# applied-ai-lab/genesis

Hardware: AMD Instinct MI355X
Metric: training images/sec (fwd+bwd+GECO step), GENESIS-V2 K=7 64x64 (higher is better)
Workload: dtype f32

## Files before the change

### genesis_amd/csrc/gx_wino.hip

```cpp
#include <stdlib.h>

#include "gx_common.h"

namespace {

constexpr int WKC = 8;
constexpr int WTH = 4, WTW = 8;
constexpr int WNT = WTH * WTW;
constexpr int PR = 2 * WTH + 2, PC = 2 * WTW + 2;
constexpr int PLANE = 10;
constexpr int PPITCH = PR * 2 * PLANE;
constexpr int RAW_FLOATS = WKC * PPITCH;
constexpr int V_FLOATS = 16 * WKC * WNT;
constexpr int RAW_PER_THREAD = (WKC * PR * PC + 255) / 256;

struct WinoGeom {
    int N, K, M;
    int K1, M1;
    int Kpad, Mpad;
    int H, W;
    int tiles_h, tiles_w;
    const float* xam0; const float* xam1;
    int xn0, xn1;
};
// ... 224 lines not shown
#pragma unroll
        for (int a = 0; a < 4; ++a)
#pragma unroll
            for (int b = 0; b < 2; ++b)
#pragma unroll
                for (int c = 0; c < 16; ++c) sacc += acc[a][b][c];
        outp[out_n + (size_t)(m0 - mbase + (tid >> 2)) * HW + (size_t)R0 * g.W + C0 + (tid & 3)] = sacc;
        return;
    }
#pragma unroll
    for (int mi = 0; mi < 2; ++mi) {
        __syncthreads();
#pragma unroll
        for (int r4 = 0; r4 < 4; ++r4)
#pragma unroll
            for (int e = 0; e < 4; ++e) {
                const int row = e + 8 * r4 + 4 * kh;
                const int rg = 4 * r4 + e;
                const float q0 = acc[0][mi][rg] + acc[1][mi][rg] + acc[2][mi][rg];
                const float q1 = acc[1][mi][rg] - acc[2][mi][rg] - acc[3][mi][rg];
                E[((wave * 2 + 0) * 32 + row) * 32 + bn] = q0;
                E[((wave * 2 + 1) * 32 + row) * 32 + bn] = q1;
            }
        __syncthreads();
#pragma unroll
        for (int j = 0; j < 4; ++j) {
            const int ml = (tid >> 5) + 8 * j;
            const int m = m0 + mi * 32 + ml;
            if (m >= g.M) continue;
            const int ty = tt >> 3, tx = tt & 7;
            float q[4][2];
#pragma unroll
            for (int xi = 0; xi < 4; ++xi) {
                q[xi][0] = E[((xi * 2 + 0) * 32 + ml) * 32 + tt];
                q[xi][1] = E[((xi * 2 + 1) * 32 + ml) * 32 + tt];
            }
            float2 y0, y1;
            y0.x = q[0][0] + q[1][0] + q[2][0];
            y0.y = q[0][1] + q[1][1] + q[2][1];
            y1.x = q[1][0] - q[2][0] - q[3][0];
            y1.y = q[1][1] - q[2][1] - q[3][1];
            float* o = outp + out_n + (size_t)(m - mbase) * HW + (size_t)(R0 + 2 * ty) * g.W + C0 + 2 * tx;
            *reinterpret_cast<float2*>(o) = y0;
            *reinterpret_cast<float2*>(o + g.W) = y1;
        }
    }
}

#ifndef GX_WH_ABL
#define GX_WH_ABL 0
#endif
constexpr int HKC = 16;
typedef __bf16 w_bf16x8 __attribute__((ext_vector_type(8)));
typedef float w_f32x16 __attribute__((ext_vector_type(16)));

__device__ __forceinline__ void wino_split8(const float (&v)[8], w_bf16x8& ph, w_bf16x8& pm, w_bf16x8& pl) {
#pragma unroll
    for (int e = 0; e < 8; ++e) {
        const __bf16 h = (__bf16)v[e];
        const float r1 = v[e] - (float)h;
        const __bf16 m = (__bf16)r1;
        ph[e] = h; pm[e] = m; pl[e] = (__bf16)(r1 - (float)m);
    }
}

typedef _Float16 w_f16x8 __attribute__((ext_vector_type(8)));
typedef float w_f32x2 __attribute__((ext_vector_type(2)));
typedef _Float16 w_f16x2 __attribute__((ext_vector_type(2)));
typedef unsigned w_u32x4 __attribute__((ext_vector_type(4)));
__device__ __forceinline__ void wino_split8_f16(const float (&v)[8], float sc, w_bf16x8& ph, w_bf16x8& pl) {
    w_u32x4 h, l;
#pragma unroll
    for (int i = 0; i < 4; ++i) {
        const float s0 = v[2 * i] * sc, s1 = v[2 * i + 1] * sc;
        const float h0 = __builtin_bit_cast(float, __builtin_bit_cast(unsigned, s0) & 0xFFFFE000u);
        const float h1 = __builtin_bit_cast(float, __builtin_bit_cast(unsigned, s1) & 0xFFFFE000u);
        h[i] = __builtin_bit_cast(unsigned, __builtin_convertvector(w_f32x2{h0, h1}, w_f16x2));
        l[i] = __builtin_bit_cast(unsigned, __builtin_convertvector(w_f32x2{s0 - h0, s1 - h1}, w_f16x2));
    }
    ph = __builtin_bit_cast(w_bf16x8, h); pl = __builtin_bit_cast(w_bf16x8, l);
}

enum { WPF_B6 = 0, WPF_F3 = 1, WPF_B1 = 2 };
template <int NB, int PF = WPF_B6> struct WHCfg {
    static constexpr int TROWS = 4 * NB;
    static constexpr int PRH = 2 * TROWS + 2;
    static constexpr int USED = PRH * 20;
    static constexpr int PITCH = NB == 1 ? 256 : 384;
    static constexpr int ROUNDS = (USED + 255) / 256;
    static constexpr int RAW_FLOATS = HKC * PITCH;
    static constexpr int NSETS = NB == 1 ? 2 : 4;
    static constexpr int LOOK = NB == 1 ? 1 : 2;
    static constexpr size_t LDS_BYTES = 2 * RAW_FLOATS * 4 > 32768 ? 2 * RAW_FLOATS * 4 : 32768;
    static constexpr int NP = PF == WPF_B1 ? 1 : (PF == WPF_F3 ? 2 : 3);
    static constexpr int POSB = (PF == WPF_B1 ? 1 : 3) * 2048;
};

template <int NB, int PF>
__global__ void __launch_bounds__(256, NB == 1 ? 2 : 1)
wino_conv_h_kernel(const float* __restrict__ in, const float* __restrict__ in2, const unsigned* __restrict__ U,
                   float* __restrict__ out, float* __restrict__ out2, const WinoGeom g) {
    using C = WHCfg<NB, PF>;
    constexpr bool F16 = PF == WPF_F3, B1 = PF == WPF_B1;
    constexpr int NP = C::NP, POSB = C::POSB;
    constexpr int PITCH = C::PITCH, NSETS = C::NSETS, LOOK = C::LOOK;
    extern __shared__ __attribute__((aligned(16))) float lds[];
    float* raw = lds;
    const int tid = threadIdx.x, lane = tid & 63, wave = tid >> 6;

    const int xcd_l = gx_xcd_tile(blockIdx.x + blockIdx.y * gridDim.x, gridDim.x * gridDim.y);
    const int my = xcd_l % (int)gridDim.y;
    int tile = xcd_l / (int)gridDim.y;
    const int tw_i = tile % g.tiles_w; tile /= g.tiles_w;
    const int th_i = tile % g.tiles_h; tile /= g.tiles_h;
    const int n = tile;
    const int R0 = th_i * (2 * C::TROWS), C0 = tw_i * (2 * WTW);
    const int m0 = my * 64;
    const int HW = g.H * g.W;
    const int Ka = g.K1 < g.K ? g.K1 : g.K, Kb = g.K - Ka;
    const float* in_n = in + (size_t)n * Ka * HW;
    const float* in2_n = in2 + (size_t)n * Kb * HW;
    const int nchunks = g.Kpad / HKC;

    int voff[C::ROUNDS];
#pragma unroll
    for (int r = 0; r < C::ROUNDS; ++r) {
        const int p = tid + 256 * r;
        voff[r] = 0x40000000;
        if (p < C::USED) {
            const int pr = p / 20, rem = p - pr * 20, par = rem / 10, idx = rem - par * 10;
            const int rr = R0 - 1 + pr, cc = C0 - 1 + 2 * idx + par;
            if (idx < 9 && rr >= 0 && rr < g.H && cc >= 0 && cc < g.W) voff[r] = (rr * g.W + cc) * 4;
        }
    }
    auto stage = [&](int k0, float* rbuf) {
        const bool second = k0 >= g.K1;
        const int kr = second ? k0 - g.K1 : k0, left = (second ? Kb : Ka) - kr;
        const __amdgpu_buffer_rsrc_t rs = __builtin_amdgcn_make_buffer_rsrc(
            const_cast<float*>((second ? in2_n : in_n) + (size_t)kr * HW), 0, left > 0 ? left * HW * 4 : 0, 0x00020000);
        float* dst = rbuf + __builtin_amdgcn_readfirstlane(wave) * 64;
#pragma unroll
        for (int q = 0; q < HKC; ++q)
#pragma unroll
            for (int r = 0; r < C::ROUNDS; ++r)
                if (r == 0 || wave < (PITCH - 256) / 64)
                    __builtin_amdgcn_raw_ptr_buffer_load_lds(rs, (__attribute__((address_space(3))) void*)(dst + q * PITCH + r * 256),
                                                             4, voff[r] + q * HW * 4, 0, 0, 0);
    };

    const int bn = lane & 31, kh = lane >> 5;
    const int tx = bn & 7;
    const int ra = wave == 0 ? 0 : (wave == 2 ? 2 : 1), rb = wave == 3 ? 3 : (wave == 2 ? 1 : 2);
    const float sgn = wave == 1 ? 1.f : -1.f;
    int ta_off[NB], tb_off[NB];
#pragma unroll
    for (int nb = 0; nb < NB; ++nb) {
        const int ty = (bn >> 3) + 4 * nb;
        ta_off[nb] = (8 * kh) * PITCH + (2 * ty + ra) * 20 + tx;
        tb_off[nb] = (8 * kh) * PITCH + (2 * ty + rb) * 20 + tx;
    }

    const char* Uw = reinterpret_cast<const char*>(U) + ((size_t)my * nchunks * 16 + 4 * wave) * POSB + lane * 16;
    auto load_a = [&](w_bf16x8 (&a)[2][3], int c, int nu) {
        const char* p = Uw + ((size_t)c * 16 + nu) * POSB;
#pragma unroll
        for (int pc = 0; pc < NP; ++pc)
#pragma unroll
            for (int mi = 0; mi < 2; ++mi)
                a[mi][pc] = *reinterpret_cast<const w_bf16x8*>(p + (pc * 2 + mi) * 1024);
    };

    w_f32x16 acc[4][2][NB];
#pragma unroll
    for (int a = 0; a < 4; ++a)
#pragma unroll
        for (int b = 0; b < 2; ++b)
#pragma unroll
            for (int nb = 0; nb < NB; ++nb)
#pragma unroll
                for (int c = 0; c < 16; ++c) acc[a][b][nb][c] = 0.f;

    w_bf16x8 as[NSETS][2][3];
    float scV = 1.f;
    int f16_back = 0;
    if constexpr (F16) {
        float xm = 0.f;
        for (int i = lane; i < g.xn0; i += 64) xm = fmaxf(xm, fabsf(g.xam0[i]));
        for (int i = lane; i < g.xn1; i += 64) xm = fmaxf(xm, fabsf(g.xam1[i]));
#pragma unroll
        for (int of = 32; of >= 1; of >>= 1) xm = fmaxf(xm, __shfl_xor(xm, of, 64));
        const int eV = gx_f16_scale_exp(4.f * xm);
        const float wam = *reinterpret_cast<const float*>(reinterpret_cast<const char*>(U) + gx_kq_h_amax_off(g.Kpad, g.Mpad, 16));
        const int eU = gx_f16_scale_exp(2.25f * wam);
        scV = ldexpf(1.f, eV);
        f16_back = -(eU + eV);
    }
#ifdef GX_WH_STAGGER
    if (((blockIdx.x + gridDim.x * blockIdx.y) >> 8) & 1)
        for (int i = 0; i < GX_WH_STAGGER; ++i) __builtin_amdgcn_s_sleep(1);
#endif
    stage(0, raw);
#pragma unroll
    for (int i = 0; i < LOOK; ++i) load_a(as[i], 0, i);

    for (int c = 0; c < nchunks; ++c) {
        __builtin_amdgcn_s_waitcnt(0x0f70);
        __syncthreads();
        if (c + 1 < nchunks && !(GX_WH_ABL & 8)) stage((c + 1) * HKC, raw + ((c + 1) & 1) * C::RAW_FLOATS);
        const float* rbuf = raw + (c & 1) * C::RAW_FLOATS;
        float t[NB][8][4];
#pragma unroll
        for (int nb = 0; nb < NB; ++nb)
#pragma unroll
            for (int ch = 0; ch < 8; ++ch) {
                const float* pa = rbuf + ta_off[nb] + ch * PITCH;
                const float* pb = rbuf + tb_off[nb] + ch * PITCH;
#pragma unroll
                for (int j = 0; j < 4; ++j) t[nb][ch][j] = fmaf(sgn, pb[(j & 1) * 10 + (j >> 1)], pa[(j & 1) * 10 + (j >> 1)]);
            }
#pragma unroll
        for (int nu = 0; nu < 4; ++nu) {
            w_bf16x8 (&acur)[2][3] = as[nu % NSETS];
            if (!(GX_WH_ABL & 2)) {
                constexpr int dummy = 0; (void)dummy;
                const int pn = nu + LOOK;
                if (pn < 4) load_a(as[pn % NSETS], c, pn);
                else if (c + 1 < nchunks) load_a(as[pn % NSETS], c + 1, pn - 4);
            }
            w_bf16x8 b[NB][3];
#pragma unroll
            for (int nb = 0; nb < NB; ++nb) {
                float v[8];
#pragma unroll
                for (int ch = 0; ch < 8; ++ch)
                    v[ch] = nu == 0 ? t[nb][ch][0] - t[nb][ch][2]
                                    : (nu == 1 ? t[nb][ch][1] + t[nb][ch][2] : (nu == 2 ? t[nb][ch][2] - t[nb][ch][1] : t[nb][ch][1] - t[nb][ch][3]));
                if (GX_WH_ABL & 4) { b[nb][0] = acur[0][0]; b[nb][1] = acur[0][1]; b[nb][2] = acur[0][2]; }
                else if constexpr (B1) {
#pragma unroll
                    for (int e = 0; e < 8; ++e) b[nb][0][e] = (__bf16)v[e];
                }
                else if constexpr (F16) wino_split8_f16(v, scV, b[nb][0], b[nb][1]);
                else wino_split8(v, b[nb][0], b[nb][1], b[nb][2]);
            }
#pragma unroll
            for (int mi = 0; mi < 2; ++mi)
#pragma unroll
                for (int nb = 0; nb < NB; ++nb) {
                    w_f32x16 cc = acc[nu][mi][nb];
                    if (GX_WH_ABL & 1) { cc[0] += (float)acur[mi][0][0] * (float)b[nb][0][0] + (float)acur[mi][1][1] * (float)b[nb][1][1] + (float)acur[mi][2][2] * (float)b[nb][2][2]; acc[nu][mi][nb] = cc; continue; }
                    if constexpr (B1) {
                        acc[nu][mi][nb] = __builtin_amdgcn_mfma_f32_32x32x16_bf16(acur[mi][0], b[nb][0], cc, 0, 0, 0);
                        continue;
                    }
                    if constexpr (F16) {
                        cc = __builtin_amdgcn_mfma_f32_32x32x16_f16(__builtin_bit_cast(w_f16x8, acur[mi][1]), __builtin_bit_cast(w_f16x8, b[nb][0]), cc, 0, 0, 0);
                        cc = __builtin_amdgcn_mfma_f32_32x32x16_f16(__builtin_bit_cast(w_f16x8, acur[mi][0]), __builtin_bit_cast(w_f16x8, b[nb][1]), cc, 0, 0, 0);
                        cc = __builtin_amdgcn_mfma_f32_32x32x16_f16(__builtin_bit_cast(w_f16x8, acur[mi][0]), __builtin_bit_cast(w_f16x8, b[nb][0]), cc, 0, 0, 0);
                        acc[nu][mi][nb] = cc;
                        continue;
                    }
                    cc = __builtin_amdgcn_mfma_f32_32x32x16_bf16(acur[mi][1], b[nb][1], cc, 0, 0, 0);
                    cc = __builtin_amdgcn_mfma_f32_32x32x16_bf16(acur[mi][2], b[nb][0], cc, 0, 0, 0);
                    cc = __builtin_amdgcn_mfma_f32_32x32x16_bf16(acur[mi][0], b[nb][2], cc, 0, 0, 0);
                    cc = __builtin_amdgcn_mfma_f32_32x32x16_bf16(acur[mi][1], b[nb][0], cc, 0, 0, 0);
                    cc = __builtin_amdgcn_mfma_f32_32x32x16_bf16(acur[mi][0], b[nb][1], cc, 0, 0, 0);
                    cc = __builtin_amdgcn_mfma_f32_32x32x16_bf16(acur[mi][0], b[nb][0], cc, 0, 0, 0);
                    acc[nu][mi][nb] = cc;
                }
        }
    }

    float* E = lds;
    const int tt = tid & 31;
    const bool second_out = m0 >= g.M1;
    const int Mo = second_out ? g.M - g.M1 : (g.M1 < g.M ? g.M1 : g.M), mbase = second_out ? g.M1 : 0;
    float* const outp = second_out ? out2 : out;
    const size_t out_n = (size_t)n * Mo * HW;
#pragma unroll
    for (int mi = 0; mi < 2; ++mi)
#pragma unroll
        for (int nb = 0; nb < NB; ++nb) {
            __syncthreads();
#pragma unroll
            for (int r4 = 0; r4 < 4; ++r4)
#pragma unroll
                for (int e = 0; e < 4; ++e) {
                    const int row = e + 8 * r4 + 4 * kh;
                    const int rg = 4 * r4 + e;
                    const float q0 = acc[0][mi][nb][rg] + acc[1][mi][nb][rg] + acc[2][mi][nb][rg];
                    const float q1 = acc[1][mi][nb][rg] - acc[2][mi][nb][rg] - acc[3][mi][nb][rg];
                    E[((wave * 2 + 0) * 32 + row) * 32 + bn] = q0;
                    E[((wave * 2 + 1) * 32 + row) * 32 + bn] = q1;
                }
            __syncthreads();
#pragma unroll
            for (int j = 0; j < 4; ++j) {
                const int ml = (tid >> 5) + 8 * j;
                const int m = m0 + mi * 32 + ml;
                if (m >= g.M) continue;
                const int oy = (tt >> 3) + 4 * nb, ox = tt & 7;
                float q[4][2];
#pragma unroll
                for (int xi = 0; xi < 4; ++xi) {
                    q[xi][0] = E[((xi * 2 + 0) * 32 + ml) * 32 + tt];
                    q[xi][1] = E[((xi * 2 + 1) * 32 + ml) * 32 + tt];
                }
                float2 y0, y1;
                y0.x = q[0][0] + q[1][0] + q[2][0];
                y0.y = q[0][1] + q[1][1] + q[2][1];
                y1.x = q[1][0] - q[2][0] - q[3][0];
                y1.y = q[1][1] - q[2][1] - q[3][1];
                if constexpr (F16) {
                    y0.x = ldexpf(y0.x, f16_back); y0.y = ldexpf(y0.y, f16_back);
                    y1.x = ldexpf(y1.x, f16_back); y1.y = ldexpf(y1.y, f16_back);
                }
                float* o = outp + out_n + (size_t)(m - mbase) * HW + (size_t)(R0 + 2 * oy) * g.W + C0 + 2 * ox;
                *reinterpret_cast<float2*>(o) = y0;
                *reinterpret_cast<float2*>(o + g.W) = y1;
            }
        }
}

__device__ __forceinline__ void wino_h_store(unsigned* __restrict__ U, float v0, float v1, int m, int k, int p, int Kpad16,
                                             bool f16 = false, int f16_exp = 0, bool b1 = false) {
    unsigned short pc[2][3];
    const float v[2] = {v0, v1};
    if (b1) {
        U[gx_wino_h_word(m, k, p, 0, Kpad16, 1)] = (unsigned)__builtin_bit_cast(unsigned short, (__bf16)v0) |
                                                   ((unsigned)__builtin_bit_cast(unsigned short, (__bf16)v1) << 16);
        return;
    }
    if (f16) {
#pragma unroll
        for (int e = 0; e < 2; ++e) {
            const float ws = ldexpf(v[e], f16_exp);
            const _Float16 h = (_Float16)ws;
            pc[e][0] = __builtin_bit_cast(unsigned short, h);
            pc[e][1] = __builtin_bit_cast(unsigned short, (_Float16)(ws - (float)h));
        }
#pragma unroll
        for (int q = 0; q < 2; ++q) U[gx_wino_h_word(m, k, p, q, Kpad16)] = (unsigned)pc[0][q] | ((unsigned)pc[1][q] << 16);
        return;
    }
#pragma unroll
    for (int e = 0; e < 2; ++e) {
        const __bf16 h = (__bf16)v[e];
        const float r1 = v[e] - (float)h;
        const __bf16 mm = (__bf16)r1;
        const __bf16 l = (__bf16)(r1 - (float)mm);
        pc[e][0] = __builtin_bit_cast(unsigned short, h);
        pc[e][1] = __builtin_bit_cast(unsigned short, mm);
        pc[e][2] = __builtin_bit_cast(unsigned short, l);
    }
#pragma unroll
    for (int q = 0; q < 3; ++q) U[gx_wino_h_word(m, k, p, q, Kpad16)] = (unsigned)pc[0][q] | ((unsigned)pc[1][q] << 16);
}

__global__ void wino_pack_h_kernel(const float* __restrict__ w, unsigned* __restrict__ U, int mode, int Co, int Ci, int Kpad16,
                                   int Mpad, const float* __restrict__ amax, int b1) {
    const int total = 16 * (Kpad16 / 2) * Mpad;
    const int f16_exp = amax ? gx_f16_scale_exp(2.25f * *amax) : 0;
    for (int idx = blockIdx.x * blockDim.x + threadIdx.x; idx < total; idx += gridDim.x * blockDim.x) {
        const int m = idx % Mpad, k = 2 * ((idx / Mpad) % (Kpad16 / 2)), p = idx / (Mpad * (Kpad16 / 2));
        wino_h_store(U, gx_wino_u_value(w, mode, Co, Ci, m, k, p), gx_wino_u_value(w, mode, Co, Ci, m, k + 1, p), m, k, p, Kpad16,
                     amax != nullptr, f16_exp, b1 != 0);
    }
}

__global__ void __launch_bounds__(1024)
wino_pair_amax_kernel(const float* __restrict__ w1, const float* __restrict__ w2, int n1, int n2, float* __restrict__ tf,
                      float* __restrict__ td) {
    const float r = gx_wg1024_amax(blockIdx.x == 0 ? w1 : w2, blockIdx.x == 0 ? n1 : n2);
    if (threadIdx.x == 0) { tf[1 + blockIdx.x] = r; td[1 + blockIdx.x] = r; }
}
__global__ void wino_pack_pair_h_kernel(const float* __restrict__ w1, const float* __restrict__ w2, unsigned* __restrict__ Uf,
                                        unsigned* __restrict__ Ud, int Co1, int Co2, int Ci, int KpadF, int MpadF, int KpadD,
                                        int MpadD, int f16, int b1) {
    const int totF = 16 * (KpadF / 2) * MpadF, totD = 16 * (KpadD / 2) * MpadD;
    int f16_exp = 0;
    if (f16) {
        float* tf = reinterpret_cast<float*>(reinterpret_cast<char*>(Uf) + gx_kq_h_amax_off(KpadF, MpadF, 16));
        float* td = reinterpret_cast<float*>(reinterpret_cast<char*>(Ud) + gx_kq_h_amax_off(KpadD, MpadD, 16));
        const float am = fmaxf(tf[1], tf[2]);
        f16_exp = gx_f16_scale_exp(2.25f * am);
        if (blockIdx.x == 0 && threadIdx.x == 0) { tf[0] = am; td[0] = am; }
    }
    for (int idx = blockIdx.x * blockDim.x + threadIdx.x; idx < totF + totD; idx += gridDim.x * blockDim.x) {
        if (idx < totF) {
            const int m = idx % MpadF, k = 2 * ((idx / MpadF) % (KpadF / 2)), p = idx / (MpadF * (KpadF / 2));
            float v[2];
#pragma unroll
            for (int e = 0; e < 2; ++e)
                v[e] = m < Co1 ? gx_wino_u_value(w1, 0, Co1, Ci, m, k + e, p) : gx_wino_u_value(w2, 0, Co2, Ci, m - Co1, k + e, p);
            wino_h_store(Uf, v[0], v[1], m, k, p, KpadF, f16 != 0, f16_exp, b1 != 0);
        } else {
            const int i = idx - totF;
            const int m = i % MpadD, k = 2 * ((i / MpadD) % (KpadD / 2)), p = i / (MpadD * (KpadD / 2));
            float v[2];
#pragma unroll
            for (int e = 0; e < 2; ++e)
                v[e] = k + e < Co1 ? gx_wino_u_value(w1, 1, Co1, Ci, m, k + e, p) : gx_wino_u_value(w2, 1, Co2, Ci, m, k + e - Co1, p);
            wino_h_store(Ud, v[0], v[1], m, k, p, KpadD, f16 != 0, f16_exp, b1 != 0);
        }
    }
}

}

static int g_wino_h = -1;
bool gx_wino_h_on() {
    if (g_wino_h < 0) {
        const int lv = gx_env_matmul_level();
        const char* env = getenv("GENESIS_WINO_BF16X6");
        g_wino_h = lv >= 0 ? (lv > 0 ? 1 : 0) : ((env && env[0] == '0') ? 0 : 1);
    }
    return g_wino_h == 1;
}
static int g_wino_b1 = -1;
bool gx_wino_b1_on(void) {
    if (g_wino_b1 < 0) g_wino_b1 = gx_env_matmul_level() == 2 ? 1 : 0;
    return g_wino_b1 == 1 && gx_wino_h_on();
}

static double g_wino_flops_f16 = 0.0, g_wino_flops_all = 0.0;
static int g_wino_f16 = -1;
static bool wino_f16_on() {
    if (g_wino_f16 < 0) {
        const int lv = gx_env_matmul_level();
        const char* env = getenv("GENESIS_WINO_F16X3");
        g_wino_f16 = lv >= 0 ? (lv == 1 ? 1 : 0) : ((env && env[0] == '0') ? 0 : 1);
    }
    return g_wino_f16 == 1 && gx_wino_h_on() && !gx_wino_b1_on();
}
int gx_wino_mode_now(void) { return !gx_wino_h_on() ? 0 : (gx_wino_b1_on() ? 3 : (wino_f16_on() ? 2 : 1)); }
namespace { struct WinoHint { const float* p0; const float* p1; int n0, n1; }; thread_local WinoHint t_wino_hint = {nullptr, nullptr, 0, 0}; }
constexpr int kWinoAmaxMax = 1536;
bool gx_wino_f16_pending(void) { return wino_f16_on() && t_wino_hint.p0 && t_wino_hint.n0 > 0 && t_wino_hint.n0 + t_wino_hint.n1 <= kWinoAmaxMax; }
bool gx_conv_input_hint(const float** p0, int* n0, const float** p1, int* n1) {
    if (!t_wino_hint.p0 || t_wino_hint.n0 <= 0) return false;
    *p0 = t_wino_hint.p0; *n0 = t_wino_hint.n0; *p1 = t_wino_hint.p1; *n1 = t_wino_hint.n1;
    return true;
}
extern "C" double gx_wino_f16_share(void) { return g_wino_flops_all > 0.0 ? g_wino_flops_f16 / g_wino_flops_all : 0.0; }
extern "C" int gx_conv_input_amax(const float* p0, int n0, const float* p1, int n1) {
    t_wino_hint.p0 = (p0 && n0 > 0) ? p0 : nullptr; t_wino_hint.n0 = t_wino_hint.p0 ? n0 : 0;
    t_wino_hint.p1 = (t_wino_hint.p0 && p1 && n1 > 0) ? p1 : nullptr; t_wino_hint.n1 = t_wino_hint.p1 ? n1 : 0;
    return GX_OK;
}

static bool wino_shape_ok(int N, int K, int M, int H, int W) {
    return N > 0 && K >= 16 && M >= 16 && H >= 8 && W >= 16 && (H % 8) == 0 && (W % 16) == 0 && H * W <= 32768;
}

static int g_wino_mode = -1;

bool gx_wino_eligible(int N, int K, int M, int H, int W) {
    if (g_wino_mode < 0) {
        const char* env = getenv("GENESIS_WINOGRAD");
        g_wino_mode = env ? (env[0] == '0' ? 0 : (env[0] == '2' ? 2 : 1)) : 1;
    }
    if (g_wino_mode == 0 || !wino_shape_ok(N, K, M, H, W)) return false;
    static const char* small_env = getenv("GENESIS_WINO_SMALL");
    const int wgs = N * (H / 8) * (W / 16) * gx_ceil_div(M, 64);
    return g_wino_mode == 2 || wgs >= 256 || (wgs >= 64 && K <= 32 && N >= 16 && !(small_env && small_env[0] == '0'));
}

static int wino_launch(const float* in, const float* in2, int K1, const float* U, float* out, float* out2, int M1, int N,
                       int K, int M, int H, int W, hipStream_t s) {
    const bool h = gx_wino_h_on();
    const bool f16 = gx_wino_f16_pending();
    const bool b1 = gx_wino_b1_on();
    WinoGeom g;
    g.xam0 = f16 ? t_wino_hint.p0 : nullptr; g.xn0 = f16 ? t_wino_hint.n0 : 0;
    g.xam1 = f16 ? t_wino_hint.p1 : nullptr; g.xn1 = f16 ? t_wino_hint.n1 : 0;
    t_wino_hint = WinoHint{nullptr, nullptr, 0, 0};
    g.N = N; g.H = H; g.W = W; g.K = K; g.M = M;
    g.Kpad = gx_round_up(K, h ? HKC : WKC);
    g.Mpad = gx_round_up(M, 64);
    g.K1 = in2 ? K1 : g.Kpad;
    g.M1 = out2 ? M1 : g.Mpad;
    if (!in2) in2 = in;
    if (!out2) out2 = out;
    static const char* nb_env = getenv("GENESIS_WINO_NB");
    const int nb = (h && !f16 && !b1 && (H % 16) == 0 && nb_env && nb_env[0] == '2') ? 2 : 1;
    g.tiles_h = H / (2 * WTH * nb);
    g.tiles_w = W / (2 * WTW);
    static bool attr_set = false;
    const size_t lds = h ? (nb == 2 ? WHCfg<2>::LDS_BYTES : WHCfg<1>::LDS_BYTES)
                         : (size_t)(2 * RAW_FLOATS + 2 * V_FLOATS) * sizeof(float);
    if (!attr_set) {
        (void)hipFuncSetAttribute(reinterpret_cast<const void*>(&wino_conv_kernel),
                                  hipFuncAttributeMaxDynamicSharedMemorySize, 160 * 1024);
        (void)hipFuncSetAttribute(reinterpret_cast<const void*>(&wino_conv_h_kernel<1, WPF_B6>),
                                  hipFuncAttributeMaxDynamicSharedMemorySize, 160 * 1024);
        (void)hipFuncSetAttribute(reinterpret_cast<const void*>(&wino_conv_h_kernel<1, WPF_F3>),
                                  hipFuncAttributeMaxDynamicSharedMemorySize, 160 * 1024);
        (void)hipFuncSetAttribute(reinterpret_cast<const void*>(&wino_conv_h_kernel<1, WPF_B1>),
                                  hipFuncAttributeMaxDynamicSharedMemorySize, 160 * 1024);
        (void)hipFuncSetAttribute(reinterpret_cast<const void*>(&wino_conv_h_kernel<2, WPF_B6>),
                                  hipFuncAttributeMaxDynamicSharedMemorySize, 160 * 1024);
        attr_set = true;
    }
    {
        const double flops = 2.0 * N * (double)M * K * 9 * H * W;
        if (h) { g_wino_flops_all += flops; if (f16 && nb == 1) g_wino_flops_f16 += flops; }
        const double bytes = 4.0 * ((double)N * K * H * W + (double)N * M * H * W + 9.0 * K * M);
        GxProf pf(KID_WINO, s, flops, bytes);
        if (h && nb == 2)
            hipLaunchKernelGGL((wino_conv_h_kernel<2, WPF_B6>), dim3(N * g.tiles_h * g.tiles_w, g.Mpad / 64), dim3(256), lds, s, in, in2,
                               reinterpret_cast<const unsigned*>(U), out, out2, g);
        else if (h && b1)
            hipLaunchKernelGGL((wino_conv_h_kernel<1, WPF_B1>), dim3(N * g.tiles_h * g.tiles_w, g.Mpad / 64), dim3(256), lds, s, in, in2,
                               reinterpret_cast<const unsigned*>(U), out, out2, g);
        else if (h && f16)
            hipLaunchKernelGGL((wino_conv_h_kernel<1, WPF_F3>), dim3(N * g.tiles_h * g.tiles_w, g.Mpad / 64), dim3(256), lds, s, in, in2,
                               reinterpret_cast<const unsigned*>(U), out, out2, g);
        else if (h)
            hipLaunchKernelGGL((wino_conv_h_kernel<1, WPF_B6>), dim3(N * g.tiles_h * g.tiles_w, g.Mpad / 64), dim3(256), lds, s, in, in2,
                               reinterpret_cast<const unsigned*>(U), out, out2, g);
        else
        hipLaunchKernelGGL(wino_conv_kernel, dim3(N * g.tiles_h * g.tiles_w, g.Mpad / 64), dim3(256), lds, s, in, in2, U,
                           out, out2, g);
    }
    GX_CHECK_LAUNCH("winograd conv3x3");
    return GX_OK;
}

int gx_wino_launch(const float* in, const float* U, float* out, int N, int K, int M, int H, int W, hipStream_t s) {
    return wino_launch(in, nullptr, 0, U, out, nullptr, 0, N, K, M, H, W, s);
}

extern "C" {

int gx_conv3x3_wino_supported(int N, int Cin, int Cout, int H, int W) { return wino_shape_ok(N, Cin, Cout, H, W); }

int gx_conv3x3_wino_policy(int mode) {
    GX_CHECK_ARG(mode >= 0 && mode <= 2, "gx_conv3x3_wino_policy: mode must be 0, 1 or 2");
    g_wino_mode = mode;
    return GX_OK;
}

static size_t wino_u_bytes(int K, int M) {
    const size_t f = (size_t)16 * gx_round_up(K, 8) * gx_round_up(M, 64) * sizeof(float);
    const size_t h = gx_wino_h_bytes(gx_round_up(K, HKC), gx_round_up(M, 64)) + 16384;
    return f > h ? f : h;
}

int gx_wino_precision(int mode) {
    GX_CHECK_ARG(mode >= -1 && mode <= 3, "gx_wino_precision: mode must be 0 (fp32 matrix pipe), 1 (bf16 pipe, six piece products), 2 (as 1, "
                                          "three fp16 piece products where the input's maxima are handed in), 3 (as 1, one bf16 piece per "
                                          "operand) or -1 (the environment's default)");
    if (mode < 0) { g_wino_h = -1; g_wino_f16 = -1; g_wino_b1 = -1; return GX_OK; }
    g_wino_h = mode ? 1 : 0;
    g_wino_f16 = mode == 2 ? 1 : 0;
    g_wino_b1 = mode == 3 ? 1 : 0;
    return GX_OK;
}

size_t gx_conv3x3_wino_ws_bytes(int N, int Cin, int Cout, int H, int W) {
    (void)N; (void)H; (void)W;
    const int c = Cin > Cout ? Cin : Cout;
    return wino_u_bytes(c, c);
}

int gx_conv3x3_wino(const float* x, const float* w, float* y, int N, int Cin, int Cout, int H, int W, int mode,
                    void* ws, size_t ws_bytes, gx_stream_t stream) {
    GX_CHECK_ARG(x && w && y && ws, "gx_conv3x3_wino: null pointer");
    GX_CHECK_ARG(mode == 0 || mode == 1, "gx_conv3x3_wino: mode must be 0 (forward) or 1 (data gradient)");
    GX_CHECK_ARG(wino_shape_ok(N, Cin, Cout, H, W),
                 "gx_conv3x3_wino: needs H %% 8 == 0, W %% 16 == 0, channels >= 16 (N=%d Cin=%d Cout=%d H=%d W=%d)", N, Cin,
                 Cout, H, W);
    GX_CHECK_ARG(ws_bytes >= gx_conv3x3_wino_ws_bytes(N, Cin, Cout, H, W), "gx_conv3x3_wino: workspace too small");
    hipStream_t s = (hipStream_t)stream;
    const int K = mode == 0 ? Cin : Cout, M = mode == 0 ? Cout : Cin;
    const bool h = gx_wino_h_on();
    const bool f16 = gx_wino_f16_pending();
    const bool b1 = gx_wino_b1_on();
    const int Kpad = gx_round_up(K, h ? HKC : WKC), Mpad = gx_round_up(M, 64);
    float* U = (float*)ws;
    float* trailer = reinterpret_cast<float*>(reinterpret_cast<char*>(U) + gx_kq_h_amax_off(Kpad, Mpad, 16));
    if (f16) {
        const int rc = gx_kq_weight_amax_launch(w, Cout * Cin * 9, trailer, s);
        if (rc) return rc;
    }
    {
        const int total = 16 * Kpad * Mpad;
        GxProf pf(KID_PACK_WEIGHTS, s, 0.0, 8.0 * total);
        if (h)
            hipLaunchKernelGGL(wino_pack_h_kernel, dim3(gx_ceil_div(total / 2, 256)), dim3(256), 0, s, w, (unsigned*)U, mode, Cout,
                               Cin, Kpad, Mpad, f16 ? (const float*)trailer : (const float*)nullptr, b1 ? 1 : 0);
        else
        hipLaunchKernelGGL(wino_pack_kernel, dim3(gx_ceil_div(total, 256)), dim3(256), 0, s, w, U, mode, Cout, Cin, Kpad,
                           Mpad);
    }
    GX_CHECK_LAUNCH("gx_conv3x3_wino(pack)");
    return gx_wino_launch(x, U, y, N, K, M, H, W, s);
}

int gx_conv3x3_pair_supported(int N, int Cin, int Co1, int Co2, int H, int W) {
    return Co1 > 0 && Co2 > 0 && wino_shape_ok(N, Cin, Co1 + Co2, H, W) && Co1 % 64 == 0;
}

size_t gx_conv3x3_pair_ws_bytes(int N, int Cin, int Co1, int Co2, int H, int W) {
    (void)N; (void)H; (void)W;
    const int Co = Co1 + Co2;
// ... 63 lines not shown
```

Before: 11930.

## Stream Winograd weight fragments through an LDS ring via async buffer loads

Weight fragments for the half-precision Winograd conv kernel were loaded from global memory straight into registers. They now go through a per-wave LDS ring using buffer_load_lds, with explicit vmcnt waits and a barrier that waits on counters inline. This is meant to hide weight-load latency and cut register pressure so two workgroups fit per CU. The experimental NB=2 tile variant and its env switch are removed, and an ablation path for the epilogue is added. The cost is extra LDS per workgroup and reliance on hand-counted vmcnt values, which must stay correct for the kernel to be right.

```diff
diff --git a/genesis_amd/csrc/gx_wino.hip b/genesis_amd/csrc/gx_wino.hip
--- a/genesis_amd/csrc/gx_wino.hip
+++ b/genesis_amd/csrc/gx_wino.hip
@@ -330,31 +330,38 @@
 }
 
 enum { WPF_B6 = 0, WPF_F3 = 1, WPF_B1 = 2 };
-template <int NB, int PF = WPF_B6> struct WHCfg {
-    static constexpr int TROWS = 4 * NB;
-    static constexpr int PRH = 2 * TROWS + 2;
+template <int PF = WPF_B6> struct WHCfg {
+    static constexpr int PRH = 10;
     static constexpr int USED = PRH * 20;
-    static constexpr int PITCH = NB == 1 ? 256 : 384;
-    static constexpr int ROUNDS = (USED + 255) / 256;
+    static constexpr int PITCH = 256;
     static constexpr int RAW_FLOATS = HKC * PITCH;
-    static constexpr int NSETS = NB == 1 ? 2 : 4;
-    static constexpr int LOOK = NB == 1 ? 1 : 2;
-    static constexpr size_t LDS_BYTES = 2 * RAW_FLOATS * 4 > 32768 ? 2 * RAW_FLOATS * 4 : 32768;
     static constexpr int NP = PF == WPF_B1 ? 1 : (PF == WPF_F3 ? 2 : 3);
     static constexpr int POSB = (PF == WPF_B1 ? 1 : 3) * 2048;
+    static constexpr int PIECES = 2 * NP;
+    static constexpr int LOOK = NP == 3 ? 2 : 3;
+    static constexpr int RING_FLOATS = 4 * LOOK * PIECES * 256;
+    static constexpr size_t LDS_BYTES = (size_t)(2 * RAW_FLOATS + RING_FLOATS) * 4;
+    static_assert(LDS_BYTES <= 80 * 1024 && 2 * RAW_FLOATS * 4 >= 32768, "two workgroups per CU; the exchange buffer fits the patches");
 };
 
-template <int NB, int PF>
-__global__ void __launch_bounds__(256, NB == 1 ? 2 : 1)
+template <int N> __device__ __forceinline__ void wh_wait_vm() { asm volatile("s_waitcnt vmcnt(%0)" ::"n"(N) : "memory"); }
+__device__ __forceinline__ void wh_wait_lgkm0() { asm volatile("s_waitcnt lgkmcnt(0)" ::: "memory"); }
+template <int N> __device__ __forceinline__ void wh_barrier() {
+    asm volatile("s_waitcnt vmcnt(%0) lgkmcnt(0)\n\ts_barrier" ::"n"(N) : "memory");
+}
+
+template <int PF>
+__global__ void __launch_bounds__(256, 2)
 wino_conv_h_kernel(const float* __restrict__ in, const float* __restrict__ in2, const unsigned* __restrict__ U,
                    float* __restrict__ out, float* __restrict__ out2, const WinoGeom g) {
-    using C = WHCfg<NB, PF>;
+    using C = WHCfg<PF>;
     constexpr bool F16 = PF == WPF_F3, B1 = PF == WPF_B1;
-    constexpr int NP = C::NP, POSB = C::POSB;
-    constexpr int PITCH = C::PITCH, NSETS = C::NSETS, LOOK = C::LOOK;
+    constexpr int NP = C::NP, POSB = C::POSB, PITCH = C::PITCH, LOOK = C::LOOK, PIECES = C::PIECES;
     extern __shared__ __attribute__((aligned(16))) float lds[];
     float* raw = lds;
     const int tid = threadIdx.x, lane = tid & 63, wave = tid >> 6;
+    const int wave_u = __builtin_amdgcn_readfirstlane(wave);
+    float* ring = lds + 2 * C::RAW_FLOATS + wave_u * (LOOK * PIECES * 256);
 
     const int xcd_l = gx_xcd_tile(blockIdx.x + blockIdx.y * gridDim.x, gridDim.x * gridDim.y);
     const int my = xcd_l % (int)gridDim.y;
@@ -362,7 +369,7 @@
     const int tw_i = tile % g.tiles_w; tile /= g.tiles_w;
     const int th_i = tile % g.tiles_h; tile /= g.tiles_h;
     const int n = tile;
-    const int R0 = th_i * (2 * C::TROWS), C0 = tw_i * (2 * WTW);
+    const int R0 = th_i * (2 * WTH), C0 = tw_i * (2 * WTW);
     const int m0 = my * 64;
     const int HW = g.H * g.W;
     const int Ka = g.K1 < g.K ? g.K1 : g.K, Kb = g.K - Ka;
@@ -370,65 +377,65 @@
     const float* in2_n = in2 + (size_t)n * Kb * HW;
     const int nchunks = g.Kpad / HKC;
 
-    int voff[C::ROUNDS];
-#pragma unroll
-    for (int r = 0; r < C::ROUNDS; ++r) {
-        const int p = tid + 256 * r;
-        voff[r] = 0x40000000;
-        if (p < C::USED) {
-            const int pr = p / 20, rem = p - pr * 20, par = rem / 10, idx = rem - par * 10;
-            const int rr = R0 - 1 + pr, cc = C0 - 1 + 2 * idx + par;
-            if (idx < 9 && rr >= 0 && rr < g.H && cc >= 0 && cc < g.W) voff[r] = (rr * g.W + cc) * 4;
-        }
+    int voff = 0x40000000;
+    if (tid < C::USED) {
+        const int pr = tid / 20, rem = tid - pr * 20, par = rem / 10, idx = rem - par * 10;
+        const int rr = R0 - 1 + pr, cc = C0 - 1 + 2 * idx + par;
+        if (idx < 9 && rr >= 0 && rr < g.H && cc >= 0 && cc < g.W) voff = (rr * g.W + cc) * 4;
     }
     auto stage = [&](int k0, float* rbuf) {
         const bool second = k0 >= g.K1;
         const int kr = second ? k0 - g.K1 : k0, left = (second ? Kb : Ka) - kr;
         const __amdgpu_buffer_rsrc_t rs = __builtin_amdgcn_make_buffer_rsrc(
             const_cast<float*>((second ? in2_n : in_n) + (size_t)kr * HW), 0, left > 0 ? left * HW * 4 : 0, 0x00020000);
-        float* dst = rbuf + __builtin_amdgcn_readfirstlane(wave) * 64;
+        float* dst = rbuf + wave_u * 64;
 #pragma unroll
         for (int q = 0; q < HKC; ++q)
-#pragma unroll
-            for (int r = 0; r < C::ROUNDS; ++r)
-                if (r == 0 || wave < (PITCH - 256) / 64)
-                    __builtin_amdgcn_raw_ptr_buffer_load_lds(rs, (__attribute__((address_space(3))) void*)(dst + q * PITCH + r * 256),
-                                                             4, voff[r] + q * HW * 4, 0, 0, 0);
+            __builtin_amdgcn_raw_ptr_buffer_load_lds(rs, (__attribute__((address_space(3))) void*)(dst + q * PITCH), 4,
+                                                     voff + q * HW * 4, 0, 0, 0);
     };
 
+    const char* Um = reinterpret_cast<const char*>(U) + (size_t)my * nchunks * 16 * POSB;
+    const int uvoff = 4 * wave * POSB + lane * 16;
+    auto fill = [&](int q) {
+        const int c = q >> 2, nu = q & 3;
+        const __amdgpu_buffer_rsrc_t rs = __builtin_amdgcn_make_buffer_rsrc(const_cast<char*>(Um + (size_t)c * 16 * POSB), 0,
+                                                                            c < nchunks ? 16 * POSB : 0, 0x00020000);
+        float* dst = ring + (q % LOOK) * (PIECES * 256);
+#pragma unroll
+        for (int pc = 0; pc < NP; ++pc)
+#pragma unroll
+            for (int mi = 0; mi < 2; ++mi)
+                __builtin_amdgcn_raw_ptr_buffer_load_lds(rs, (__attribute__((address_space(3))) void*)(dst + (pc * 2 + mi) * 256), 16,
+                                                         uvoff, nu * POSB + (pc * 2 + mi) * 1024, 0, 0);
+    };
+    auto read_a = [&](w_bf16x8 (&a)[2][3], int q) {
+        const float* src = ring + (q % LOOK) * (PIECES * 256) + lane * 4;
+#pragma unroll
+        for (int pc = 0; pc < NP; ++pc)
+#pragma unroll
+            for (int mi = 0; mi < 2; ++mi) a[mi][pc] = *reinterpret_cast<const w_bf16x8*>(src + (pc * 2 + mi) * 256);
+    };
+
+    stage(0, raw);
+#pragma unroll
+    for (int q = 0; q < LOOK; ++q) fill(q);
+
     const int bn = lane & 31, kh = lane >> 5;
-    const int tx = bn & 7;
+    const int tx = bn & 7, ty = bn >> 3;
     const int ra = wave == 0 ? 0 : (wave == 2 ? 2 : 1), rb = wave == 3 ? 3 : (wave == 2 ? 1 : 2);
     const float sgn = wave == 1 ? 1.f : -1.f;
-    int ta_off[NB], tb_off[NB];
-#pragma unroll
-    for (int nb = 0; nb < NB; ++nb) {
-        const int ty = (bn >> 3) + 4 * nb;
-        ta_off[nb] = (8 * kh) * PITCH + (2 * ty + ra) * 20 + tx;
-        tb_off[nb] = (8 * kh) * PITCH + (2 * ty + rb) * 20 + tx;
-    }
-
-    const char* Uw = reinterpret_cast<const char*>(U) + ((size_t)my * nchunks * 16 + 4 * wave) * POSB + lane * 16;
-    auto load_a = [&](w_bf16x8 (&a)[2][3], int c, int nu) {
-        const char* p = Uw + ((size_t)c * 16 + nu) * POSB;
-#pragma unroll
-        for (int pc = 0; pc < NP; ++pc)
-#pragma unroll
-            for (int mi = 0; mi < 2; ++mi)
-                a[mi][pc] = *reinterpret_cast<const w_bf16x8*>(p + (pc * 2 + mi) * 1024);
-    };
-
-    w_f32x16 acc[4][2][NB];
+    const int ta_off = (8 * kh) * PITCH + (2 * ty + ra) * 20 + tx;
+    const int tb_off = (8 * kh) * PITCH + (2 * ty + rb) * 20 + tx;
+
+    w_f32x16 acc[4][2];
 #pragma unroll
     for (int a = 0; a < 4; ++a)
 #pragma unroll
         for (int b = 0; b < 2; ++b)
 #pragma unroll
-            for (int nb = 0; nb < NB; ++nb)
-#pragma unroll
-                for (int c = 0; c < 16; ++c) acc[a][b][nb][c] = 0.f;
-
-    w_bf16x8 as[NSETS][2][3];
+            for (int c = 0; c < 16; ++c) acc[a][b][c] = 0.f;
+
     float scV = 1.f;
     int f16_back = 0;
     if constexpr (F16) {
@@ -447,127 +454,128 @@
     if (((blockIdx.x + gridDim.x * blockIdx.y) >> 8) & 1)
         for (int i = 0; i < GX_WH_STAGGER; ++i) __builtin_amdgcn_s_sleep(1);
 #endif
-    stage(0, raw);
-#pragma unroll
-    for (int i = 0; i < LOOK; ++i) load_a(as[i], 0, i);
-
     for (int c = 0; c < nchunks; ++c) {
-        __builtin_amdgcn_s_waitcnt(0x0f70);
-        __syncthreads();
-        if (c + 1 < nchunks && !(GX_WH_ABL & 8)) stage((c + 1) * HKC, raw + ((c + 1) & 1) * C::RAW_FLOATS);
+        wh_barrier<LOOK * PIECES>();
+        if (!(GX_WH_ABL & 8)) stage((c + 1) * HKC, raw + ((c + 1) & 1) * C::RAW_FLOATS);
         const float* rbuf = raw + (c & 1) * C::RAW_FLOATS;
-        float t[NB][8][4];
-#pragma unroll
-        for (int nb = 0; nb < NB; ++nb)
-#pragma unroll
-            for (int ch = 0; ch < 8; ++ch) {
-                const float* pa = rbuf + ta_off[nb] + ch * PITCH;
-                const float* pb = rbuf + tb_off[nb] + ch * PITCH;
-#pragma unroll
-                for (int j = 0; j < 4; ++j) t[nb][ch][j] = fmaf(sgn, pb[(j & 1) * 10 + (j >> 1)], pa[(j & 1) * 10 + (j >> 1)]);
+        float t[8][4];
+#pragma unroll
+        for (int ch = 0; ch < 8; ++ch) {
+            const float* pa = rbuf + ta_off + ch * PITCH;
+            const float* pb = rbuf + tb_off + ch * PITCH;
+#pragma unroll
+            for (int j = 0; j < 4; ++j) t[ch][j] = fmaf(sgn, pb[(j & 1) * 10 + (j >> 1)], pa[(j & 1) * 10 + (j >> 1)]);
+        }
+#pragma unroll
+        for (int nu = 0; nu < 4; ++nu) {
+            const int q = 4 * c + nu;
+            if (nu < LOOK) wh_wait_vm<(LOOK - 1) * PIECES + HKC>();
+            else wh_wait_vm<(LOOK - 1) * PIECES>();
+            w_bf16x8 acur[2][3];
+            read_a(acur, q);
+            w_bf16x8 b[3];
+            {
+                float v[8];
+#pragma unroll
+                for (int ch = 0; ch < 8; ++ch)
+                    v[ch] = nu == 0 ? t[ch][0] - t[ch][2]
+                                    : (nu == 1 ? t[ch][1] + t[ch][2] : (nu == 2 ? t[ch][2] - t[ch][1] : t[ch][1] - t[ch][3]));
+                if (GX_WH_ABL & 4) { b[0] = acur[0][0]; b[1] = acur[0][1]; b[2] = acur[0][2]; }
+                else if constexpr (B1) {
+#pragma unroll
+                    for (int e = 0; e < 8; ++e) b[0][e] = (__bf16)v[e];
+                }
+                else if constexpr (F16) wino_split8_f16(v, scV, b[0], b[1]);
+                else wino_split8(v, b[0], b[1], b[2]);
             }
 #pragma unroll
-        for (int nu = 0; nu < 4; ++nu) {
-            w_bf16x8 (&acur)[2][3] = as[nu % NSETS];
-            if (!(GX_WH_ABL & 2)) {
-                constexpr int dummy = 0; (void)dummy;
-                const int pn = nu + LOOK;
-                if (pn < 4) load_a(as[pn % NSETS], c, pn);
-                else if (c + 1 < nchunks) load_a(as[pn % NSETS], c + 1, pn - 4);
+            for (int mi = 0; mi < 2; ++mi) {
+                w_f32x16 cc = acc[nu][mi];
+                if (GX_WH_ABL & 1) { cc[0] += (float)acur[mi][0][0] * (float)b[0][0] + (float)acur[mi][1][1] * (float)b[1][1] + (float)acur[mi][2][2] * (float)b[2][2]; acc[nu][mi] = cc; continue; }
+                if constexpr (B1) {
+                    acc[nu][mi] = __builtin_amdgcn_mfma_f32_32x32x16_bf16(acur[mi][0], b[0], cc, 0, 0, 0);
+                    continue;
+                }
+                if constexpr (F16) {
+                    cc = __builtin_amdgcn_mfma_f32_32x32x16_f16(__builtin_bit_cast(w_f16x8, acur[mi][1]), __builtin_bit_cast(w_f16x8, b[0]), cc, 0, 0, 0);
+                    cc = __builtin_amdgcn_mfma_f32_32x32x16_f16(__builtin_bit_cast(w_f16x8, acur[mi][0]), __builtin_bit_cast(w_f16x8, b[1]), cc, 0, 0, 0);
+                    cc = __builtin_amdgcn_mfma_f32_32x32x16_f16(__builtin_bit_cast(w_f16x8, acur[mi][0]), __builtin_bit_cast(w_f16x8, b[0]), cc, 0, 0, 0);
+                    acc[nu][mi] = cc;
+                    continue;
+                }
+                cc = __builtin_amdgcn_mfma_f32_32x32x16_bf16(acur[mi][1], b[1], cc, 0, 0, 0);
+                cc = __builtin_amdgcn_mfma_f32_32x32x16_bf16(acur[mi][2], b[0], cc, 0, 0, 0);
+                cc = __builtin_amdgcn_mfma_f32_32x32x16_bf16(acur[mi][0], b[2], cc, 0, 0, 0);
+                cc = __builtin_amdgcn_mfma_f32_32x32x16_bf16(acur[mi][1], b[0], cc, 0, 0, 0);
+                cc = __builtin_amdgcn_mfma_f32_32x32x16_bf16(acur[mi][0], b[1], cc, 0, 0, 0);
+                cc = __builtin_amdgcn_mfma_f32_32x32x16_bf16(acur[mi][0], b[0], cc, 0, 0, 0);
+                acc[nu][mi] = cc;
             }
-            w_bf16x8 b[NB][3];
-#pragma unroll
-            for (int nb = 0; nb < NB; ++nb) {
-                float v[8];
-#pragma unroll
-                for (int ch = 0; ch < 8; ++ch)
-                    v[ch] = nu == 0 ? t[nb][ch][0] - t[nb][ch][2]
-                                    : (nu == 1 ? t[nb][ch][1] + t[nb][ch][2] : (nu == 2 ? t[nb][ch][2] - t[nb][ch][1] : t[nb][ch][1] - t[nb][ch][3]));
-                if (GX_WH_ABL & 4) { b[nb][0] = acur[0][0]; b[nb][1] = acur[0][1]; b[nb][2] = acur[0][2]; }
-                else if constexpr (B1) {
-#pragma unroll
-                    for (int e = 0; e < 8; ++e) b[nb][0][e] = (__bf16)v[e];
-                }
-                else if constexpr (F16) wino_split8_f16(v, scV, b[nb][0], b[nb][1]);
-                else wino_split8(v, b[nb][0], b[nb][1], b[nb][2]);
-            }
-#pragma unroll
-            for (int mi = 0; mi < 2; ++mi)
-#pragma unroll
-                for (int nb = 0; nb < NB; ++nb) {
-                    w_f32x16 cc = acc[nu][mi][nb];
-                    if (GX_WH_ABL & 1) { cc[0] += (float)acur[mi][0][0] * (float)b[nb][0][0] + (float)acur[mi][1][1] * (float)b[nb][1][1] + (float)acur[mi][2][2] * (float)b[nb][2][2]; acc[nu][mi][nb] = cc; continue; }
-                    if constexpr (B1) {
-                        acc[nu][mi][nb] = __builtin_amdgcn_mfma_f32_32x32x16_bf16(acur[mi][0], b[nb][0], cc, 0, 0, 0);
-                        continue;
-                    }
-                    if constexpr (F16) {
-                        cc = __builtin_amdgcn_mfma_f32_32x32x16_f16(__builtin_bit_cast(w_f16x8, acur[mi][1]), __builtin_bit_cast(w_f16x8, b[nb][0]), cc, 0, 0, 0);
-                        cc = __builtin_amdgcn_mfma_f32_32x32x16_f16(__builtin_bit_cast(w_f16x8, acur[mi][0]), __builtin_bit_cast(w_f16x8, b[nb][1]), cc, 0, 0, 0);
-                        cc = __builtin_amdgcn_mfma_f32_32x32x16_f16(__builtin_bit_cast(w_f16x8, acur[mi][0]), __builtin_bit_cast(w_f16x8, b[nb][0]), cc, 0, 0, 0);
-                        acc[nu][mi][nb] = cc;
-                        continue;
-                    }
-                    cc = __builtin_amdgcn_mfma_f32_32x32x16_bf16(acur[mi][1], b[nb][1], cc, 0, 0, 0);
-                    cc = __builtin_amdgcn_mfma_f32_32x32x16_bf16(acur[mi][2], b[nb][0], cc, 0, 0, 0);
-                    cc = __builtin_amdgcn_mfma_f32_32x32x16_bf16(acur[mi][0], b[nb][2], cc, 0, 0, 0);
-                    cc = __builtin_amdgcn_mfma_f32_32x32x16_bf16(acur[mi][1], b[nb][0], cc, 0, 0, 0);
-                    cc = __builtin_amdgcn_mfma_f32_32x32x16_bf16(acur[mi][0], b[nb][1], cc, 0, 0, 0);
-                    cc = __builtin_amdgcn_mfma_f32_32x32x16_bf16(acur[mi][0], b[nb][0], cc, 0, 0, 0);
-                    acc[nu][mi][nb] = cc;
-                }
-        }
-    }
-
+            wh_wait_lgkm0();
+            if (!(GX_WH_ABL & 2)) fill(q + LOOK);
+            if constexpr (B1) __builtin_amdgcn_sched_barrier(0);
+        }
+    }
+
+    wh_wait_vm<0>();
     float* E = lds;
     const int tt = tid & 31;
     const bool second_out = m0 >= g.M1;
     const int Mo = second_out ? g.M - g.M1 : (g.M1 < g.M ? g.M1 : g.M), mbase = second_out ? g.M1 : 0;
     float* const outp = second_out ? out2 : out;
     const size_t out_n = (size_t)n * Mo * HW;
-#pragma unroll
-    for (int mi = 0; mi < 2; ++mi)
-#pragma unroll
-        for (int nb = 0; nb < NB; ++nb) {
-            __syncthreads();
-#pragma unroll
-            for (int r4 = 0; r4 < 4; ++r4)
-#pragma unroll
-                for (int e = 0; e < 4; ++e) {
-                    const int row = e + 8 * r4 + 4 * kh;
-                    const int rg = 4 * r4 + e;
-                    const float q0 = acc[0][mi][nb][rg] + acc[1][mi][nb][rg] + acc[2][mi][nb][rg];
-                    const float q1 = acc[1][mi][nb][rg] - acc[2][mi][nb][rg] - acc[3][mi][nb][rg];
-                    E[((wave * 2 + 0) * 32 + row) * 32 + bn] = q0;
-                    E[((wave * 2 + 1) * 32 + row) * 32 + bn] = q1;
-                }
-            __syncthreads();
-#pragma unroll
-            for (int j = 0; j < 4; ++j) {
-                const int ml = (tid >> 5) + 8 * j;
-                const int m = m0 + mi * 32 + ml;
-                if (m >= g.M) continue;
-                const int oy = (tt >> 3) + 4 * nb, ox = tt & 7;
-                float q[4][2];
-#pragma unroll
-                for (int xi = 0; xi < 4; ++xi) {
-                    q[xi][0] = E[((xi * 2 + 0) * 32 + ml) * 32 + tt];
-                    q[xi][1] = E[((xi * 2 + 1) * 32 + ml) * 32 + tt];
-                }
-                float2 y0, y1;
-                y0.x = q[0][0] + q[1][0] + q[2][0];
-                y0.y = q[0][1] + q[1][1] + q[2][1];
-                y1.x = q[1][0] - q[2][0] - q[3][0];
-                y1.y = q[1][1] - q[2][1] - q[3][1];
-                if constexpr (F16) {
-                    y0.x = ldexpf(y0.x, f16_back); y0.y = ldexpf(y0.y, f16_back);
-                    y1.x = ldexpf(y1.x, f16_back); y1.y = ldexpf(y1.y, f16_back);
-                }
-                float* o = outp + out_n + (size_t)(m - mbase) * HW + (size_t)(R0 + 2 * oy) * g.W + C0 + 2 * ox;
-                *reinterpret_cast<float2*>(o) = y0;
-                *reinterpret_cast<float2*>(o + g.W) = y1;
+    if (GX_WH_ABL & 16) {
+        float sacc = 0.f;
+#pragma unroll
+        for (int a = 0; a < 4; ++a)
+#pragma unroll
+            for (int b = 0; b < 2; ++b)
+#pragma unroll
+                for (int c = 0; c < 16; ++c) sacc += acc[a][b][c];
+        outp[out_n + (size_t)R0 * g.W + C0 + (tid & 15)] = sacc;
+        return;
+    }
+#pragma unroll
+    for (int mi = 0; mi < 2; ++mi) {
+        __syncthreads();
+#pragma unroll
+        for (int r4 = 0; r4 < 4; ++r4)
+#pragma unroll
+            for (int e = 0; e < 4; ++e) {
+                const int row = e + 8 * r4 + 4 * kh;
+                const int rg = 4 * r4 + e;
+                const float q0 = acc[0][mi][rg] + acc[1][mi][rg] + acc[2][mi][rg];
+                const float q1 = acc[1][mi][rg] - acc[2][mi][rg] - acc[3][mi][rg];
+                E[((wave * 2 + 0) * 32 + row) * 32 + bn] = q0;
+                E[((wave * 2 + 1) * 32 + row) * 32 + bn] = q1;
             }
-        }
+        __syncthreads();
+#pragma unroll
+        for (int j = 0; j < 4; ++j) {
+            const int ml = (tid >> 5) + 8 * j;
+            const int m = m0 + mi * 32 + ml;
+            if (m >= g.M) continue;
+            const int oy = tt >> 3, ox = tt & 7;
+            float q[4][2];
+#pragma unroll
+            for (int xi = 0; xi < 4; ++xi) {
+                q[xi][0] = E[((xi * 2 + 0) * 32 + ml) * 32 + tt];
+                q[xi][1] = E[((xi * 2 + 1) * 32 + ml) * 32 + tt];
+            }
+            float2 y0, y1;
+            y0.x = q[0][0] + q[1][0] + q[2][0];
+            y0.y = q[0][1] + q[1][1] + q[2][1];
+            y1.x = q[1][0] - q[2][0] - q[3][0];
+            y1.y = q[1][1] - q[2][1] - q[3][1];
+            if constexpr (F16) {
+                y0.x = ldexpf(y0.x, f16_back); y0.y = ldexpf(y0.y, f16_back);
+                y1.x = ldexpf(y1.x, f16_back); y1.y = ldexpf(y1.y, f16_back);
+            }
+            float* o = outp + out_n + (size_t)(m - mbase) * HW + (size_t)(R0 + 2 * oy) * g.W + C0 + 2 * ox;
+            *reinterpret_cast<float2*>(o) = y0;
+            *reinterpret_cast<float2*>(o + g.W) = y1;
+        }
+    }
 }
 
 __device__ __forceinline__ void wino_h_store(unsigned* __restrict__ U, float v0, float v1, int m, int k, int p, int Kpad16,
@@ -730,46 +738,39 @@
     g.M1 = out2 ? M1 : g.Mpad;
     if (!in2) in2 = in;
     if (!out2) out2 = out;
-    static const char* nb_env = getenv("GENESIS_WINO_NB");
-    const int nb = (h && !f16 && !b1 && (H % 16) == 0 && nb_env && nb_env[0] == '2') ? 2 : 1;
-    g.tiles_h = H / (2 * WTH * nb);
+    g.tiles_h = H / (2 * WTH);
     g.tiles_w = W / (2 * WTW);
     static bool attr_set = false;
-    const size_t lds = h ? (nb == 2 ? WHCfg<2>::LDS_BYTES : WHCfg<1>::LDS_BYTES)
+    const size_t lds = h ? (b1 ? WHCfg<WPF_B1>::LDS_BYTES : (f16 ? WHCfg<WPF_F3>::LDS_BYTES : WHCfg<WPF_B6>::LDS_BYTES))
                          : (size_t)(2 * RAW_FLOATS + 2 * V_FLOATS) * sizeof(float);
     if (!attr_set) {
         (void)hipFuncSetAttribute(reinterpret_cast<const void*>(&wino_conv_kernel),
                                   hipFuncAttributeMaxDynamicSharedMemorySize, 160 * 1024);
-        (void)hipFuncSetAttribute(reinterpret_cast<const void*>(&wino_conv_h_kernel<1, WPF_B6>),
+        (void)hipFuncSetAttribute(reinterpret_cast<const void*>(&wino_conv_h_kernel<WPF_B6>),
                                   hipFuncAttributeMaxDynamicSharedMemorySize, 160 * 1024);
-        (void)hipFuncSetAttribute(reinterpret_cast<const void*>(&wino_conv_h_kernel<1, WPF_F3>),
+        (void)hipFuncSetAttribute(reinterpret_cast<const void*>(&wino_conv_h_kernel<WPF_F3>),
                                   hipFuncAttributeMaxDynamicSharedMemorySize, 160 * 1024);
-        (void)hipFuncSetAttribute(reinterpret_cast<const void*>(&wino_conv_h_kernel<1, WPF_B1>),
-                                  hipFuncAttributeMaxDynamicSharedMemorySize, 160 * 1024);
-        (void)hipFuncSetAttribute(reinterpret_cast<const void*>(&wino_conv_h_kernel<2, WPF_B6>),
+        (void)hipFuncSetAttribute(reinterpret_cast<const void*>(&wino_conv_h_kernel<WPF_B1>),
                                   hipFuncAttributeMaxDynamicSharedMemorySize, 160 * 1024);
         attr_set = true;
     }
     {
         const double flops = 2.0 * N * (double)M * K * 9 * H * W;
-        if (h) { g_wino_flops_all += flops; if (f16 && nb == 1) g_wino_flops_f16 += flops; }
+        if (h) { g_wino_flops_all += flops; if (f16) g_wino_flops_f16 += flops; }
         const double bytes = 4.0 * ((double)N * K * H * W + (double)N * M * H * W + 9.0 * K * M);
         GxProf pf(KID_WINO, s, flops, bytes);
-        if (h && nb == 2)
-            hipLaunchKernelGGL((wino_conv_h_kernel<2, WPF_B6>), dim3(N * g.tiles_h * g.tiles_w, g.Mpad / 64), dim3(256), lds, s, in, in2,
-                               reinterpret_cast<const unsigned*>(U), out, out2, g);
-        else if (h && b1)
-            hipLaunchKernelGGL((wino_conv_h_kernel<1, WPF_B1>), dim3(N * g.tiles_h * g.tiles_w, g.Mpad / 64), dim3(256), lds, s, in, in2,
-                               reinterpret_cast<const unsigned*>(U), out, out2, g);
+        const dim3 grid(N * g.tiles_h * g.tiles_w, g.Mpad / 64);
+        if (h && b1)
+            hipLaunchKernelGGL((wino_conv_h_kernel<WPF_B1>), grid, dim3(256), lds, s, in, in2, reinterpret_cast<const unsigned*>(U),
+                               out, out2, g);
         else if (h && f16)
-            hipLaunchKernelGGL((wino_conv_h_kernel<1, WPF_F3>), dim3(N * g.tiles_h * g.tiles_w, g.Mpad / 64), dim3(256), lds, s, in, in2,
-                               reinterpret_cast<const unsigned*>(U), out, out2, g);
+            hipLaunchKernelGGL((wino_conv_h_kernel<WPF_F3>), grid, dim3(256), lds, s, in, in2, reinterpret_cast<const unsigned*>(U),
+                               out, out2, g);
         else if (h)
-            hipLaunchKernelGGL((wino_conv_h_kernel<1, WPF_B6>), dim3(N * g.tiles_h * g.tiles_w, g.Mpad / 64), dim3(256), lds, s, in, in2,
-                               reinterpret_cast<const unsigned*>(U), out, out2, g);
+            hipLaunchKernelGGL((wino_conv_h_kernel<WPF_B6>), grid, dim3(256), lds, s, in, in2, reinterpret_cast<const unsigned*>(U),
+                               out, out2, g);
         else
-        hipLaunchKernelGGL(wino_conv_kernel, dim3(N * g.tiles_h * g.tiles_w, g.Mpad / 64), dim3(256), lds, s, in, in2, U,
-                           out, out2, g);
+        hipLaunchKernelGGL(wino_conv_kernel, grid, dim3(256), lds, s, in, in2, U, out, out2, g);
     }
     GX_CHECK_LAUNCH("winograd conv3x3");
     return GX_OK;
```

New measurement: 11920, median of 4. No clear change (-0.1%).
